# TMmichi/mujoco_jaco

Hardware: AMD Instinct MI355X
Metric: env-steps/sec at batch 65 536 (full Jaco + gripper + contacts) (higher is better)
Workload: dtype f32

## Files before the change

### __graft_entry__.py

```python
import os
import subprocess
import sys

ROOT = os.path.dirname(os.path.abspath(__file__))
CSRC = os.path.join(ROOT, "mujoco_jaco_amd", "csrc")
HIPCC = os.environ.get("HIPCC", "/opt/rocm/bin/hipcc")


D12 = ["-DJNB=13", "-DJNV=18", "-DJNQ=19", "-DJB0=12", "-DJB1=18", "-DJNSENS=64", "-DJMAXCHAIN=8", "-DJMAXDESC=12", "-DJMAXINNER=9"]
D30 = ["-DJNB=20", "-DJNV=30", "-DJNQ=32", "-DJB0=18", "-DJB1=24", "-DJNU=18", "-DJNSENS=40", "-DJMAXGEOM=128", "-DJMAXPAIR=3584", "-DJMAXINNER=12",
       "-DJMAXMPAIR=192", "-DJACO_LIGHT_WAVES=2"]


FLAGS = ["--offload-arch=gfx950", "-O3", "-std=c++17", "-fno-hip-fp32-correctly-rounded-divide-sqrt", "-fno-slp-vectorize",
         "-fgpu-flush-denormals-to-zero", "-fPIC", "-Rpass-analysis=kernel-resource-usage", "-I", os.path.join(CSRC, "include")]
NKERNEL_TU = 14


def _variant_jobs(name, extra):
    bdir = os.path.join(ROOT, "build", name)
    os.makedirs(bdir, exist_ok=True)
    jobs, objs = [], []
    for tu in list(range(NKERNEL_TU)) + [-1]:
        src = "jaco_env.hip" if tu < 0 else "kernels.hip"
# ... 34 lines not shown
    while todo or running:
        while todo and len(running) < workers and not failed:
            cmd, log = todo.pop(0)
            running.append((subprocess.Popen(cmd, cwd=CSRC, stdout=open(log, "w"), stderr=subprocess.STDOUT), cmd, log))
        if failed and not running:
            break
        p, cmd, log = running.pop(0)
        if p.poll() is None:
            running.append((p, cmd, log))
            import time
            time.sleep(0.2)
            continue
        if p.returncode == 0:
            open(log[:-4] + ".cmd", "w").write(" ".join(cmd))
        if p.returncode != 0:
            failed.append((cmd, log))
            for q, _, _ in running:
                q.terminate()
            for q, _, _ in running:
                q.wait()
            running = []
    if failed:
        cmd, log = failed[0]
        raise RuntimeError("hipcc failed: %s\n%s" % (" ".join(cmd), open(log).read()[-4000:]))
    for link in links:
        subprocess.check_call(link, cwd=CSRC)


VARIANTS = {
    "default": [],
    "d12": D12,
    "d30": D30,
    "prof": ["-DJACO_PROFILE_STAGES"],
}


def build():
    build_libs({k: v for k, v in VARIANTS.items() if k != "prof" or os.environ.get("JACO_BUILD_PROF") == "1"})
    subprocess.check_call(["make", "-s", "-C", os.path.join(ROOT, "oracle")])
    subprocess.check_call(["make", "-s", "-C", os.path.join(ROOT, "tests", "emu")])
    subprocess.check_call(["make", "-s", "-C", os.path.join(ROOT, "tests", "emu_osc")])
    subprocess.check_call(["make", "-s", "-C", os.path.join(ROOT, "tests", "emu_osc_task")])
    subprocess.check_call(["make", "-s", "-C", os.path.join(ROOT, "tests", "emu_joint")])
    if os.path.isdir("/root/reference/env_script/assets/jaco2") and not os.path.exists(
            os.path.join(ROOT, "mujoco_jaco_amd", "assets", "jaco2_curtain_torque.jacomdl")):
        subprocess.check_call([sys.executable, "-m", "mujoco_jaco_amd.modelc.compile"], cwd=ROOT)
    sys.path.insert(0, ROOT)
    import mujoco_jaco_amd
    from mujoco_jaco_amd import _lib
    _lib.load()
    _lib.load("_d12")
    _lib.load("_d30")


def smoke():
    sys.path.insert(0, ROOT)
    sys.path.insert(0, os.path.join(ROOT, "tests"))
    import numpy as np
    import torch
    from mujoco_jaco_amd import workload
    from mujoco_jaco_amd.modelc import blob
    from mujoco_jaco_amd.physics import BatchedMujoco
    from oracle_binding import Oracle

    B, nsub = 64, 20
    M = blob.load(os.path.join(ROOT, "mujoco_jaco_amd", "assets", "jaco2_curtain_torque.jacomdl"))
    q = workload.reset_states(M["qpos0"], B, seed=7, f32_draws=True)
    c = workload.random_ctrl(B, seed=8, scale=0.2).astype(np.float32).astype(np.float64)
    env = BatchedMujoco(B, device=0)
    dev = env.device
    env.set_state(torch.tensor(q, dtype=torch.float32, device=dev), None, None)
# ... 31 lines not shown
```

### mujoco_jaco_amd/csrc/physics_kernel.h

```cpp
#pragma once
#include <stdint.h>
#include <jaco/model_dev.h>
#include <jaco/wave_ops.h>

#ifndef JACO_WRENCH
#define JACO_WRENCH 0
#endif
template <int MAXEFC_, int MAXCON_, int MAXCAND_, bool CONTACT_ = true>
struct JacoCaps {
  static_assert(MAXEFC_ % 64 == 0, "rows are dealt out 64 at a time (one per lane): the row capacity must be a multiple of 64");
  static constexpr bool WRENCH = CONTACT_ && JACO_WRENCH != 0;
  static_assert(WRENCH || JMAXGEOM != 64 || JNV != 21 || MAXCAND_ <= MAXEFC_ * 25 - 520 - 256 - 576, "default layout: the candidate list must fit behind the geom poses in the constraint-row area");
  static constexpr int MAXEFC = MAXEFC_, MAXCON = MAXCON_, MAXCAND = MAXCAND_, NR = MAXEFC_ / 64;
  static constexpr bool CONTACT = CONTACT_;
  static constexpr int JROWS = CONTACT_ ? MAXEFC_ : (JNB <= 16 ? 16 : 32), NGEOM = CONTACT_ ? JMAXGEOM : 1;
  static_assert(CONTACT_ || JNB <= 32, "limit rows of the contact-free instantiation");
};
#if JACO_WRENCH
typedef JacoCaps<128, 32, 240> JacoLight;
#else
typedef JacoCaps<64, 32, 240> JacoLight;
#endif
typedef JacoCaps<128, 32, 512> JacoMedium;
#ifndef JACO_HEAVY_ROWS
// ... 14 lines not shown
#define JFLAG_CON_OVERFLOW 1u
#define JFLAG_EFC_OVERFLOW 2u
#define JFLAG_CAND_OVERFLOW 4u
#define JFLAG_NAN 8u
#define JFLAG_SOLVER_MAXITER 16u
#define JFLAG_HEAVY_TIER 32u
#define JFLAG_BAIL_CAUSE_SHIFT 8
#define JFLAG_TIER_RETURN 128u

#define JMINVAL 1e-15f
#define JTASK_FLOATS 40

#define JPROF_N 16
struct JProfCtx {
  unsigned long long tprev;
  unsigned long long* row;
};
#ifdef JACO_PROFILE_STAGES
JDEV void jprof_stamp(JProfCtx& pc, int i, int lane) {
  unsigned long long t = __builtin_amdgcn_s_memtime();
  if (lane == 0 && pc.row) pc.row[i] += t - pc.tprev;
  pc.tprev = __builtin_amdgcn_s_memtime();
}
#define JSTAMP(i) jprof_stamp(pc, (i), lane)
#else
#define JSTAMP(i)
#endif
#ifdef JACO_NARROW_PROFILE
#define JSTAMP_NEWTON(i) JSTAMP(6)
#define JSTAMP_NARROW(i) JSTAMP(i)
#else
#define JSTAMP_NEWTON(i) JSTAMP(i)
#define JSTAMP_NARROW(i)
#endif

struct JacoContactRec {
  float dist, pos[3], frame[9];
  float force[6];
  int geom[2], body[2], dim;
};
#define JCONREC_WORDS 24
#define JCONREC_MAX_CAPACITY 1024
#define JSTR_(x) #x
#define JSTR(x) JSTR_(x)
static inline const char* jaco_contact_record_check(const void* rec, const int* ncon, int capacity) {
  if (!ncon || capacity < 1 || capacity > JCONREC_MAX_CAPACITY) return "needs a count buffer and 1 <= capacity <= " JSTR(JCONREC_MAX_CAPACITY);
  if ((reinterpret_cast<uintptr_t>(rec) & 15u) != 0) return "the record buffer must be 16-byte aligned";
  return nullptr;
}

enum JacoMode { JM_CTRL = 0, JM_STEP = 1, JM_FORWARD = 2, JM_HOLD = 3, JM_TAKE_ACTION = 4, JM_TERMINAL = 5, JM_PREREACH = 6 };
#define JM_REAL_STEP(m) ((m) <= JM_STEP)
#define JM_MASKED(m) ((m) == JM_FORWARD || (m) == JM_HOLD || (m) == JM_PREREACH)
#define JM_TASK_SUBSTEPS(m) ((m) == JM_STEP || (m) == JM_HOLD || (m) == JM_PREREACH)
#define JM_NO_SUBSTEP(m) ((m) == JM_TAKE_ACTION || (m) == JM_TERMINAL)

struct JacoStepArgs {
  const JacoModelDev* model;
  const float* hull;
  float* qpos;
  float* qvel;
  float* qpos_lo;
  float* qvel_lo;
  float* qacc_ws;
  const float* ctrl;
  float* sensordata;
// ... 776 lines not shown
template <class L>
JDEV void stage_limit_rows(const JacoModelDev* m, L& s, int lane, const StagePrefetch& pf) {
  bool act = false;
  float dist = 0.f, sgn = 1.f;
  int d = 0;
  if (lane < m->nbody && s.mc.b_jtype[lane] == JJ_HINGE && pf.limited) {
    float q = s.qpos[s.mc.b_qadr[lane]];
    float lo = q - pf.lo, hi = pf.hi - q;
    d = s.mc.b_dadr[lane];
    if (lo < 0.f) { act = true; dist = lo; sgn = 1.f; }
    else if (hi < 0.f) { act = true; dist = hi; sgn = -1.f; }
  }
  unsigned long long mask = wave_ballot(act);
  int r = wave_prefix_count(mask);
  if (act) {
    if (L::Caps::WRENCH) {
      for (int k = 0; k < 8; k++) s.J[r * 8 + k] = 0.f;
      s.J[r * 8] = sgn;
    } else {
      for (int k = 0; k < JNV; k++) s.J[r * JLD + k] = 0.f;
      s.J[r * JLD + d] = sgn;
    }
    float R;
    s.e_aref[r] = row_params(m->b_solref[lane], m->b_solimp[lane], dist, sgn * s.qvel[d], m->d_invweight[d], &R);
    s.e_D[r] = 1.f / R;
    s.e_con[r] = ((d < JB0 ? 1 : (d < JB1 ? 2 : 4)) << 16) | (L::Caps::WRENCH ? (JW_UNIT | (d << 19)) : 0);
  }
  if (lane == 0) { s.nefc = popc64(mask); s.nlimit = s.nefc; }
}

struct NewtonOut { float qacc, qfrc_con, qdamped; int iters; bool have_qdamped; };
#define JDAMPED_BLOCKS 1

template <int NR>
JDEV void rows_dot(const float* J, const float (&jrow)[JNV], float vk, int lane, int ne, int nv, float (&out)[NR]) {
  float vb[JNV];
#pragma unroll
  for (int k = 0; k < JNV; k++) vb[k] = wave_bcast(vk, k);
  if (NR == 1) {
    float acc = 0.f;
#pragma unroll
    for (int k = 0; k < JNV; k++) acc += jrow[k] * vb[k];
    out[0] = acc;
    return;
  }
  const float* Jr[NR];
#pragma unroll
  for (int q = 0; q < NR; q++) { int r = lane + 64 * q; Jr[q] = J + (r < ne ? r : 0) * JLD; out[q] = 0.f; }
#pragma unroll
  for (int k = 0; k < JNV; k++) {
#pragma unroll
    for (int q = 0; q < NR; q++) out[q] += Jr[q][k] * vb[k];
  }
  (void)nv;
}
JDEV float mat_vec(const float (&mrow)[JNV], float vk) {
  float vb[JNV];
#pragma unroll
  for (int k = 0; k < JNV; k++) vb[k] = wave_bcast(vk, k);
  float acc = 0.f;
#pragma unroll
  for (int k = 0; k < JNV; k++) acc += mrow[k] * vb[k];
  return acc;
}
template <int NR>
JDEV float jt_vec(const float* J, const float (&f)[NR], int ne, int lane, int nv) {
  float acc = 0.f;
  int kk = lane < nv ? lane : 0;
#pragma unroll
  for (int q = 0; q < NR; q++) {
    int n = ne - 64 * q;
    n = n > 64 ? 64 : n;
    const float* Jq = J + (64 * q) * JLD + kk;
    int rl = 0;
    for (; rl + 4 <= n; rl += 4) {
      float j0 = Jq[(rl + 0) * JLD], j1 = Jq[(rl + 1) * JLD], j2 = Jq[(rl + 2) * JLD], j3 = Jq[(rl + 3) * JLD];
      const float f0 = wave_bcast(f[q], rl), f1 = wave_bcast(f[q], rl + 1), f2 = wave_bcast(f[q], rl + 2), f3 = wave_bcast(f[q], rl + 3);
      acc += j0 * f0 + j1 * f1 + j2 * f2 + j3 * f3;
    }
    for (; rl < n; rl++) acc += Jq[rl * JLD] * wave_bcast(f[q], rl);
  }
  return lane < nv ? acc : 0.f;
}

#ifndef JACO_NEWTON_LOOKAHEAD
#define JACO_NEWTON_LOOKAHEAD 1
#endif
JDEV bool newton_next_round_is_idle(bool any_row_switched, float al, float improvement, float scale, float tol) {
  const float r = 1.f - al;
  return JACO_NEWTON_LOOKAHEAD && !any_row_switched && r * r * improvement * scale < tol;
}
template <class L>
JDEV NewtonOut stage_newton(const JacoModelDev* m, L& s, const float (&mrow)[JNV], float smooth, float hd, int lane, JProfCtx& pc) {
  (void)pc;
  constexpr int NR = L::Caps::NR, MAXEFC = L::Caps::MAXEFC;
  NewtonOut out;
  int nv = m->nv, ne = wave_uniform_i(s.nefc);
  out.qfrc_con = 0.f; out.iters = 0; out.qdamped = 0.f; out.have_qdamped = false;
  float h0[JNV];
#pragma unroll
  for (int j = 0; j < JNV; j++) h0[j] = lane < nv ? mrow[j] : (lane == j ? 1.f : 0.f);
  const int blockmask = 1 | (nv > JB0 ? 2 : 0) | (nv > JB1 ? 4 : 0);
  if (ne == 0) {
    if (m->has_damping == 1) {
      out.qacc = ldl_block0_dual(h0, smooth, hd, lane, &out.qdamped) + ldl_solve_blocks(h0, smooth, lane, blockmask & 6);
      out.have_qdamped = true;
    } else out.qacc = ldl_solve_blocks(h0, smooth, lane, blockmask);
    return out;
  }
  if (ne > MAXEFC) ne = MAXEFC;
  bool valid[NR];
  float D[NR], ar[NR], x[NR], f[NR], jp[NR];
  int blk[NR];
  float jrow[JNV];
#pragma unroll
  for (int q = 0; q < NR; q++) {
    int r = lane + 64 * q;
    valid[q] = r < ne;
    D[q] = valid[q] ? s.e_D[r] : 0.f;
    ar[q] = valid[q] ? s.e_aref[r] : 0.f;
    blk[q] = valid[q] ? (s.e_con[r] >> 16) & 7 : 0;
  }
#pragma unroll
  for (int k = 0; k < JNV; k++) jrow[k] = (NR == 1 && lane < ne) ? s.J[lane * JLD + k] : 0.f;
  float scale = 1.f / (m->meaninertia * (float)(nv > 1 ? nv : 1));
  float tol = m->tolerance;
  int rowblk = 0;
#pragma unroll
  for (int q = 0; q < NR; q++) rowblk |= blk[q];
  const int rowblocks = (wave_ballot(rowblk & 1) ? 1 : 0) | (wave_ballot(rowblk & 2) ? 2 : 0) | (wave_ballot(rowblk & 4) ? 4 : 0);
  const bool mine = lane < nv && ((lane < JB0 ? 1 : (lane < JB1 ? 2 : 4)) & rowblocks) != 0;
  float afree;
  if ((rowblocks & 1) == 0 && m->has_damping == 1) {
    afree = ldl_block0_dual(h0, smooth, hd, lane, &out.qdamped);
    out.have_qdamped = true;
    afree += ldl_solve_blocks(h0, smooth, lane, ~rowblocks & 6 & blockmask);
  } else afree = ldl_solve_blocks(h0, smooth, lane, ~rowblocks & 7 & blockmask);
  float a = mine ? s.qacc_ws[lane] : afree;
  float Ma = mat_vec(mrow, a) - smooth;
  Ma = mine ? Ma : 0.f;
  rows_dot<NR>(s.J, jrow, a, lane, ne, nv, x);
#pragma unroll
  for (int q = 0; q < NR; q++) x[q] = valid[q] ? x[q] - ar[q] : 0.f;
  JSTAMP_NEWTON(11);
#ifdef JACO_EMULATED
  if (lane == 0) emu_counter[8]++;
#endif
  int it = 0, nls = 0;
  for (; it < m->iterations; it++) {
    lane = wave_opaque_i(lane);
#ifdef JACO_EMULATED
    if (lane == 0) emu_counter[9]++;
#endif
    bool coupled = false;
#pragma unroll
    for (int q = 0; q < NR; q++) {
      f[q] = x[q] < 0.f ? -D[q] * x[q] : 0.f;
      coupled = coupled || (x[q] < 0.f && (blk[q] & (blk[q] - 1)) != 0);
    }
    bool full = wave_ballot(coupled) != 0ull;
    float* xs = NR == 1 ? s.smooth : s.e_x;
#pragma unroll
    for (int q = 0; q < NR; q++) if (valid[q]) { s.e_f[lane + 64 * q] = x[q] < 0.f ? D[q] : 0.f; xs[lane + 64 * q] = x[q]; }
    wave_sync();
    float h[JNV], jtf;
    if ((rowblocks & 1) == 0) {
      acc16x16 C;
      acc_zero(C);
      const int uq = lane >> 4, col = lane & 15;
      const float cj = col < JNV - JB0 ? 1.f : 0.f, cx = col == JNV - JB0 ? -1.f : 0.f;
      const float* jcol = s.J + JB0 + (col < JNV - JB0 ? col : 0);
      const int last = ne - 1;
      for (int r0 = 0; r0 < ne; r0 += 16) {
        float jv[4], wv[4];
#pragma unroll
        for (int u = 0; u < 4; u++) {
          const int r = r0 + 4 * u + uq, rc = r < last ? r : last;
          jv[u] = cj * jcol[rc * JLD] + cx * xs[rc];
          wv[u] = r < ne ? s.e_f[rc] : 0.f;
// ... 14 lines not shown
    } else {
    acc32x32 C;
    acc_zero(C);
    const int uh = lane >> 5, col = lane & 31;
    const float cj = col < JNV ? 1.f : 0.f, cx = col == JNV ? -1.f : 0.f;
    const float* jcol = s.J + (col < JNV ? col : 0);
    const int last = ne - 1;
    for (int r0 = 0; r0 < ne; r0 += 8) {
      float jv[4], wv[4];
#pragma unroll
      for (int u = 0; u < 4; u++) {
        const int r = r0 + 2 * u + uh, rc = r < last ? r : last;
        jv[u] = cj * jcol[rc * JLD] + cx * xs[rc];
        wv[u] = r < ne ? s.e_f[rc] : 0.f;
      }
#pragma unroll
      for (int u = 0; u < 4; u++) wave_mfma_32x32x2(jv[u], wv[u] * jv[u], C);
    }
    JSTAMP_NEWTON(12);
#pragma unroll
    for (int j2 = 0; j2 < JNV; j2++) {
      const int reg = (j2 & 3) + 4 * (j2 >> 3);
      float cv = ((j2 >> 2) & 1) ? wave_shfl(C.v[reg], (lane + 32) & 63) : C.v[reg];
      h[j2] = lane < nv ? mrow[j2] + cv : (lane == j2 ? 1.f : 0.f);
    }
    jtf = ((JNV >> 2) & 1) ? wave_shfl(C.v[(JNV & 3) + 4 * (JNV >> 3)], (lane + 32) & 63) : C.v[(JNV & 3) + 4 * (JNV >> 3)];
    }
    float grad = Ma - (lane < nv ? jtf : 0.f);
    float gn = sqrtf(wave_sum(grad * grad));
    if (gn * scale < tol) break;
    float p = !full ? ldl_solve_blocks(h, -grad, lane, rowblocks) : ((rowblocks & 1) == 0 ? ldl_block<JB0, JNV>(h, -grad, lane) : ldl_solve<true>(h, -grad, lane));
    p = lane < nv ? p : 0.f;
    JSTAMP_NEWTON(13);
    float Mp = mat_vec(mrow, p);
    float pMp, pMa;
    wave_sum2(p * Mp, p * Ma, &pMp, &pMa);
    rows_dot<NR>(s.J, jrow, p, lane, ne, nv, jp);
#pragma unroll
    for (int q = 0; q < NR; q++) jp[q] = valid[q] ? jp[q] : 0.f;
    float al = 0.f, lo = 0.f, hi = 3.0e38f, d10 = 0.f, dlo = 0.f, dhi = 0.f;
    for (int ls = 0; ls < m->ls_iterations; ls++) {
      float s1 = 0.f, s2 = 0.f;
#pragma unroll
      for (int q = 0; q < NR; q++) {
        float xa = x[q] + al * jp[q];
        s1 += xa < 0.f ? D[q] * xa * jp[q] : 0.f;
        s2 += xa < 0.f ? D[q] * jp[q] * jp[q] : 0.f;
      }
      float w1, w2;
      wave_sum2(s1, s2, &w1, &w2);
      float d1 = pMa + al * pMp + w1, d2 = pMp + w2;
      if (ls == 0) d10 = fabsf(d1);
#ifdef JACO_TRACE_LS
      if (lane == 0) printf("it %d ls %d al %.9g d1 %.6g d2 %.6g lo %.9g hi %.9g pMa %.6g pMp %.6g\n", it, ls, al, d1, d2, lo, hi, pMa, pMp);
#endif
      if (ls > 0 && fabsf(d1) <= 1e-6f * d10) break;
      if (d1 < 0.f) { lo = al; dlo = -d1; } else { hi = al; dhi = d1; }
      if (hi < 1.0e38f && fmaxf(dlo, dhi) * (hi - lo) * scale < 1e-3f * tol) break;
      const float stepn = d1 / d2;
      float nx = al - stepn;
      if (!(nx > lo && nx < hi)) nx = hi < 1.0e38f ? 0.5f * (lo + hi) : 2.f * al + 1.f;
      if (nx == al) break;
      al = nx;
      nls++;
    }
    float dc = 0.f;
    bool switched = false;
#pragma unroll
    for (int q = 0; q < NR; q++) {
      float dx = al * jp[q], xn = x[q] + dx;
      bool was = x[q] < 0.f, is = xn < 0.f;
      switched = switched || was != is;
      dc += (was && is) ? 0.5f * D[q] * dx * (2.f * x[q] + dx) : (is ? 0.5f * D[q] * xn * xn : (was ? -0.5f * D[q] * x[q] * x[q] : 0.f));
      x[q] = xn;
    }
    const bool any_switched = wave_ballot(switched) != 0ull;
    float improvement = -(al * pMa + 0.5f * al * al * pMp + wave_sum(dc));
    JSTAMP_NEWTON(14);
    a += al * p; Ma += al * Mp;
    if (improvement * scale < tol || newton_next_round_is_idle(any_switched, al, improvement, scale, tol)) { it++; break; }
  }
#pragma unroll
  for (int q = 0; q < NR; q++) f[q] = x[q] < 0.f ? -D[q] * x[q] : 0.f;
  out.qacc = a;
  out.qfrc_con = jt_vec<NR>(s.J, f, ne, lane, nv);
  out.iters = it | (nls << 8);
#pragma unroll
  for (int q = 0; q < NR; q++) if (valid[q]) s.e_f[lane + 64 * q] = f[q];
  return out;
}

struct WCol { sv S; unsigned mv; };
template <class L>
JDEV WCol wcol_load(const L& s, int col, int nv) {
  WCol c;
  const bool ok = col < nv;
  c.S = ldsv(s.cdof[ok ? col : 0]);
  if (!ok) { c.S.a = mk3(0.f, 0.f, 0.f); c.S.b = mk3(0.f, 0.f, 0.f); }
  c.mv = ok ? s.mc.b_descmask[s.mc.d_body[col]] << 1 : 0u;
  return c;
}
JDEV float wrow_entry(const WCol& c, int col, const v4& a, const v4& b, int con) {
  const float sgn = (float)((int)((c.mv >> ((con >> 24) & 31)) & 1u) - (int)((c.mv >> ((con >> 19) & 31)) & 1u));
  const float body = sgn * (a.x * c.S.a.x + a.y * c.S.a.y + a.z * c.S.a.z + a.w * c.S.b.x + b.x * c.S.b.y + b.y * c.S.b.z);
  return (con & JW_UNIT) ? (((con >> 19) & 31) == col ? a.x : 0.f) : body;
}
template <int NR, class L>
JDEV void rows_dot_w(L& s, const float (&w)[NR][6], const int (&con)[NR], float vk, int lane, int nv, int ncon, float (&out)[NR]) {
  float* vs = s.smooth + 32;
  wave_sync();
  if (lane < nv) vs[lane] = vk;
  wave_sync();
  for (int idx = lane; idx < 6 * ncon; idx += 64) {
    const int c = idx / 6, comp = idx - 6 * c, obs = s.c_ob[c];
    const int B1 = (obs >> 8) & 31, B2 = (obs >> 24) & 31;
    const unsigned m1 = B1 ? s.mc.b_chain[B1 - 1] : 0u, m2 = B2 ? s.mc.b_chain[B2 - 1] : 0u;
    const unsigned plus = m2 & ~m1;
    unsigned mask = m1 ^ m2;
    float acc = 0.f;
    while (mask) {
      const int k = __builtin_ctz(mask);
      mask &= mask - 1u;
      const float t = s.cdof[k][comp] * vs[k];
      acc += ((plus >> k) & 1u) ? t : -t;
    }
    s.c_frame[c][3 + comp] = acc;
  }
  wave_sync();
#pragma unroll
  for (int q = 0; q < NR; q++) {
    const bool unit = (con[q] & JW_UNIT) != 0;
    const float* Dc = s.c_frame[unit ? 0 : (con[q] & 255)] + 3;
    float acc = 0.f;
#pragma unroll
    for (int c = 0; c < 6; c++) acc += w[q][c] * Dc[c];
    out[q] = unit ? w[q][0] * vs[(con[q] >> 19) & 31] : acc;
  }
}

template <class L>
JDEV NewtonOut stage_newton_w(const JacoModelDev* m, L& s, const float (&mrow)[JNV], float smooth, float hd, int lane, JProfCtx& pc) {
  (void)pc;
  constexpr int NR = L::Caps::NR, MAXEFC = L::Caps::MAXEFC;
  NewtonOut out;
  const int nv = m->nv, ncon = wave_uniform_i(s.ncon), nlim = wave_uniform_i(s.nlimit);
  int ne = wave_uniform_i(s.nefc);
  out.qfrc_con = 0.f; out.iters = 0; out.qdamped = 0.f; out.have_qdamped = false;
  float h0[JNV];
#pragma unroll
  for (int j = 0; j < JNV; j++) h0[j] = lane < nv ? mrow[j] : (lane == j ? 1.f : 0.f);
  const int blockmask = 1 | (nv > JB0 ? 2 : 0) | (nv > JB1 ? 4 : 0);
  if (ne == 0) {
    if (m->has_damping == 1) {
      out.qacc = ldl_block0_dual(h0, smooth, hd, lane, &out.qdamped) + ldl_solve_blocks(h0, smooth, lane, blockmask & 6);
      out.have_qdamped = true;
    } else out.qacc = ldl_solve_blocks(h0, smooth, lane, blockmask);
    return out;
  }
  if (ne > MAXEFC) ne = MAXEFC;
  bool valid[NR];
  float D[NR], ar[NR], x[NR], f[NR], jp[NR], w[NR][6];
  int con[NR];
#pragma unroll
  for (int q = 0; q < NR; q++) {
    const int r = lane + 64 * q;
    valid[q] = r < ne;
    const int rc = valid[q] ? r : 0;
    D[q] = valid[q] ? s.e_D[rc] : 0.f;
    ar[q] = valid[q] ? s.e_aref[rc] : 0.f;
    con[q] = valid[q] ? s.e_con[rc] : 0;
    const v4 a = ld4(s.J + 8 * rc), b = ld4(s.J + 8 * rc + 4);
    w[q][0] = valid[q] ? a.x : 0.f; w[q][1] = valid[q] ? a.y : 0.f; w[q][2] = valid[q] ? a.z : 0.f;
    w[q][3] = valid[q] ? a.w : 0.f; w[q][4] = valid[q] ? b.x : 0.f; w[q][5] = valid[q] ? b.y : 0.f;
  }
// ... 129 lines not shown
#pragma unroll
    for (int q = 0; q < NR; q++) {
      float dx = al * jp[q], xn = x[q] + dx;
      bool was = x[q] < 0.f, is = xn < 0.f;
      switched = switched || was != is;
      dc += (was && is) ? 0.5f * D[q] * dx * (2.f * x[q] + dx) : (is ? 0.5f * D[q] * xn * xn : (was ? -0.5f * D[q] * x[q] * x[q] : 0.f));
      x[q] = xn;
    }
    const bool any_switched = wave_ballot(switched) != 0ull;
    float improvement = -(al * pMa + 0.5f * al * al * pMp + wave_sum(dc));
    JSTAMP_NEWTON(14);
    a += al * p; Ma += al * Mp;
    if (improvement * scale < tol || newton_next_round_is_idle(any_switched, al, improvement, scale, tol)) { it++; break; }
  }
#pragma unroll
  for (int q = 0; q < NR; q++) f[q] = x[q] < 0.f ? -D[q] * x[q] : 0.f;
  out.qacc = a;
  out.iters = it | (nls << 8);
  wave_sync();
#pragma unroll
  for (int q = 0; q < NR; q++) if (valid[q]) { s.e_f[lane + 64 * q] = f[q]; s.J[8 * (lane + 64 * q) + JW_WT] = f[q]; }
  wave_sync();
  for (int ci = lane; ci < ncon; ci += 64) {
    const int cd = s.c_dim[ci], nrow = cd == 1 ? 1 : 2 * (cd - 1), r0 = s.c_efc[ci];
    float F[6] = {0.f, 0.f, 0.f, 0.f, 0.f, 0.f};
    for (int e = 0; e < nrow; e++) {
      const v4 ra = ld4(s.J + 8 * (r0 + e)), rb = ld4(s.J + 8 * (r0 + e) + 4);
      F[0] += rb.z * ra.x; F[1] += rb.z * ra.y; F[2] += rb.z * ra.z; F[3] += rb.z * ra.w; F[4] += rb.z * rb.x; F[5] += rb.z * rb.y;
    }
#pragma unroll
    for (int c = 0; c < 6; c++) s.c_frame[ci][3 + c] = F[c];
  }
  wave_sync();
  {
    const WCol own = wcol_load(s, lane, nv);
    float acc = 0.f;
    for (int c = 0; c < ncon; c++) {
      const int obs = s.c_ob[c];
      const float sgn = (float)((int)((own.mv >> ((obs >> 24) & 31)) & 1u) - (int)((own.mv >> ((obs >> 8) & 31)) & 1u));
      const float* F = s.c_frame[c] + 3;
      acc += sgn * (F[0] * own.S.a.x + F[1] * own.S.a.y + F[2] * own.S.a.z + F[3] * own.S.b.x + F[4] * own.S.b.y + F[5] * own.S.b.z);
    }
    for (int r = 0; r < nlim; r++) {
      const int cn = s.e_con[r];
      if (((cn >> 19) & 31) == lane) acc += s.J[8 * r] * s.J[8 * r + JW_WT];
    }
    out.qfrc_con = lane < nv ? acc : 0.f;
  }
  return out;
}

template <class L>
JDEV NewtonOut stage_newton_limits(const JacoModelDev* m, L& s, const float (&mrow)[JNV], float smooth, float hd, int lane) {
  NewtonOut out;
  const int nv = m->nv, ne = wave_uniform_i(s.nefc);
  out.qfrc_con = 0.f; out.iters = 0; out.qdamped = 0.f; out.have_qdamped = false;
  float h0[JNV];
#pragma unroll
  for (int j = 0; j < JNV; j++) h0[j] = lane < nv ? mrow[j] : (lane == j ? 1.f : 0.f);
  const int blockmask = 1 | (nv > JB0 ? 2 : 0) | (nv > JB1 ? 4 : 0);
  if (ne == 0) {
    if (m->has_damping == 1) {
      out.qacc = ldl_block0_dual(h0, smooth, hd, lane, &out.qdamped) + ldl_solve_blocks(h0, smooth, lane, blockmask & 6);
      out.have_qdamped = true;
    } else out.qacc = ldl_solve_blocks(h0, smooth, lane, blockmask);
    return out;
  }
// ... 94 lines not shown
      const float e1 = q1 * cm1 + q0 * d1 + q2 * d3 - q3 * d2;
      const float e2 = q2 * cm1 + q0 * d2 - q1 * d3 + q3 * d1;
      const float e3 = q3 * cm1 + q0 * d3 + q1 * d2 - q2 * d1;
      if (comp) {
        f2 r;
        r = comp_add(q0, l0, e0, 0.f); q0 = r.hi; l0 = r.lo;
        r = comp_add(q1, l1, e1, 0.f); q1 = r.hi; l1 = r.lo;
        r = comp_add(q2, l2, e2, 0.f); q2 = r.hi; l2 = r.lo;
        r = comp_add(q3, l3, e3, 0.f); q3 = r.hi; l3 = r.lo;
      } else { q0 += e0; q1 += e1; q2 += e2; q3 += e3; }
    }
    const float r2 = fmaf(q3, q3, fmaf(q2, q2, fmaf(q1, q1, fmaf(q0, q0, -1.f)))) + 2.f * (q0 * l0 + q1 * l1 + q2 * l2 + q3 * l3);
    if (comp && fabsf(r2) < 1e-3f) {
      const float k = r2 * (-0.5f + 0.375f * r2);
      f2 r;
      r = comp_add(q0, l0, q0 * k, 0.f); q0 = r.hi; l0 = r.lo;
      r = comp_add(q1, l1, q1 * k, 0.f); q1 = r.hi; l1 = r.lo;
      r = comp_add(q2, l2, q2 * k, 0.f); q2 = r.hi; l2 = r.lo;
      r = comp_add(q3, l3, q3 * k, 0.f); q3 = r.hi; l3 = r.lo;
    } else {
      const float n = sqrtf(q0 * q0 + q1 * q1 + q2 * q2 + q3 * q3);
      if (n < JMINVAL) { q0 = 1.f; q1 = q2 = q3 = 0.f; } else { const float in = 1.f / n; q0 *= in; q1 *= in; q2 *= in; q3 *= in; }
      l0 = l1 = l2 = l3 = 0.f;
    }
    s.qpos[qa + 3] = q0; s.qpos[qa + 4] = q1; s.qpos[qa + 5] = q2; s.qpos[qa + 6] = q3;
    if (comp) { s.qpos_lo[qa + 3] = l0; s.qpos_lo[qa + 4] = l1; s.qpos_lo[qa + 5] = l2; s.qpos_lo[qa + 6] = l3; }
  }
}

#include "collision.h"
#include "env_logic.h"

template <class L>
JDEV void newton_side(const JacoModelDev* m, L& s, const float (&mrow)[JNV], float smooth, int lane, NewtonOut& out) {
  float* sd = side_buf(s);
  int ns = wave_uniform_i(s.nside);
  ns = ns < 0 ? 0 : (ns > JSIDE_ROWS ? JSIDE_ROWS : ns);
  const int nv = m->nv;
  const bool mine = lane >= JB1 && lane < JNV, vr = lane < ns;
  const int kk = mine ? lane - JB1 : 0, rr = vr ? lane : 0;
  float js[6];
#pragma unroll
  for (int k = 0; k < 6; k++) js[k] = vr ? sd[JSIDE_J + rr * 6 + k] : 0.f;
  const float D = vr ? sd[JSIDE_D + rr] : 0.f, ar = vr ? sd[JSIDE_AREF + rr] : 0.f;
  const float scale = 1.f / (m->meaninertia * (float)(nv > 1 ? nv : 1)), tol = m->tolerance;
  wave_sync();
  float a = mine ? s.qacc_ws[lane] : 0.f;
  float Ma = 0.f, x = 0.f;
#pragma unroll
  for (int j = 0; j < 6; j++) { const float aj = wave_bcast(a, JB1 + j); Ma += mrow[JB1 + j] * aj; x += js[j] * aj; }
  Ma = mine ? Ma - smooth : 0.f;
  x = vr ? x - ar : 0.f;
  float jtf = 0.f;
  int it = 0;
  for (; it < m->iterations; it++) {
    lane = wave_opaque_i(lane);
    if (vr) { sd[JSIDE_F + lane] = x < 0.f ? D : 0.f; sd[JSIDE_AREF + lane] = x < 0.f ? -D * x : 0.f; }
    wave_sync();
    float h[JNV];
#pragma unroll
    for (int j = 0; j < JNV; j++) h[j] = (j >= JB1 && mine) ? mrow[j] : 0.f;
    jtf = 0.f;
    for (int r = 0; r < ns; r++) {
      const float* Jr = sd + JSIDE_J + r * 6;
      const float jk = Jr[kk], t = sd[JSIDE_F + r] * jk;
      jtf += jk * sd[JSIDE_AREF + r];
#pragma unroll
// ... 10 lines not shown
    Mp = mine ? Mp : 0.f;
    jp = vr ? jp : 0.f;
    float pMp, pMa;
    wave_sum2(p * Mp, p * Ma, &pMp, &pMa);
    float al = 0.f, lo = 0.f, hi = 3.0e38f, d10 = 0.f, dlo = 0.f, dhi = 0.f;
    for (int ls = 0; ls < m->ls_iterations; ls++) {
      const float xa = x + al * jp;
      const float s1 = xa < 0.f ? D * xa * jp : 0.f, s2 = xa < 0.f ? D * jp * jp : 0.f;
      float w1, w2;
      wave_sum2(s1, s2, &w1, &w2);
      float d1 = pMa + al * pMp + w1, d2 = pMp + w2;
      if (ls == 0) d10 = fabsf(d1);
      if (ls > 0 && fabsf(d1) <= 1e-6f * d10) break;
      if (d1 < 0.f) { lo = al; dlo = -d1; } else { hi = al; dhi = d1; }
      if (hi < 1.0e38f && fmaxf(dlo, dhi) * (hi - lo) * scale < 1e-3f * tol) break;
      float nx = al - d1 / d2;
      if (!(nx > lo && nx < hi)) nx = hi < 1.0e38f ? 0.5f * (lo + hi) : 2.f * al + 1.f;
      if (nx == al) break;
      al = nx;
    }
    const float dx = al * jp, xn = x + dx;
    const bool was = x < 0.f, is = xn < 0.f;
    const bool any_switched = wave_ballot(was != is) != 0ull;
    const float dc = (was && is) ? 0.5f * D * dx * (2.f * x + dx) : (is ? 0.5f * D * xn * xn : (was ? -0.5f * D * x * x : 0.f));
    x = xn;
    const float improvement = -(al * pMa + 0.5f * al * al * pMp + wave_sum(dc));
    a += al * p; Ma += al * Mp;
    if (improvement * scale < tol || newton_next_round_is_idle(any_switched, al, improvement, scale, tol)) { it++; break; }
  }
  const float f = x < 0.f ? -D * x : 0.f;
  wave_sync();
  if (vr) sd[JSIDE_F + lane] = f;
  wave_sync();
  float qf = 0.f;
  for (int r = 0; r < ns; r++) qf += sd[JSIDE_J + r * 6 + kk] * sd[JSIDE_F + r];
  out.qacc = mine ? a : out.qacc;
  out.qfrc_con = mine ? qf : out.qfrc_con;
  if (it > (out.iters & 255)) out.iters = (out.iters & ~255) | (it & 255);
}

JDEV void queue_push(const JacoStepArgs& A, int t, int env, int left, int lane) {
  if (lane == 0) st_wt_i(&A.remaining[env], left);
  dev_stores_done();
  wave_sync();
  if (lane == 0) {
    int slot = jaco_atomic_inc(A.q[t].count);
    st_wt_i(&A.q[t].list[slot], env);
    dev_stores_done();
  }
}
JDEV void hint_raise(const JacoStepArgs& A, int env, int tier, int lane) {
  if (lane == 0 && A.hint) atomicMax(&A.hint[env], tier);
}

template <class L>
JDEV void stage_record(const JacoModelDev* m, L& s, JacoContactRec* rec, int* nout, int cap, int env, int lane) {
  const int ncon = L::Caps::CONTACT ? wave_uniform_i(s.ncon) : 0;
  if (lane == 0) nout[env] = ncon;
  if constexpr (L::Caps::CONTACT) {
    const int n = ncon < cap ? ncon : cap;
    for (int ci = lane; ci < n; ci += 64) {
      const int cd = s.c_dim[ci], nrow = cd == 1 ? 1 : 2 * (cd - 1), r0 = s.c_efc[ci], obs = s.c_ob[ci];
      const float* f = (SideRows<L>::on && r0 >= JSIDE_BASE) ? side_buf(s) + JSIDE_F + (r0 - JSIDE_BASE) : s.e_f + r0;
      const JacoPairParam& P = m->pair[s.c_pair[ci]];
      float fc[6] = {0.f, 0.f, 0.f, 0.f, 0.f, 0.f};
      for (int e = 0; e < nrow; e++) fc[0] += f[e];
#pragma unroll
      for (int k = 1; k < 6; k++) if (k < cd) fc[k] = P.mu[k - 1] * (f[2 * k - 2] - f[2 * k - 1]);
      const float* fr = s.c_frame[ci];
      v4* o = reinterpret_cast<v4*>(rec + (size_t)env * cap + ci);
// ... 236 lines not shown
    if (!LIGHT) {
      constexpr int LCON = TIER == 3 ? JacoHeavy::MAXCON : (TIER == 2 ? JacoMedium::MAXCON : JacoLight::MAXCON);
      constexpr int LEFC = TIER == 3 ? JacoHeavy::MAXEFC : (TIER == 2 ? JacoMedium::MAXEFC : JacoLight::MAXEFC);
      constexpr int LCAND = TIER == 3 ? JacoHeavy::MAXCAND : (TIER == 2 ? JacoMedium::MAXCAND : JacoLight::MAXCAND);
      const bool rows_fit = s.nefc <= LEFC || (TIER == 1 && SideRows<JacoLDS<JacoLight>>::on && s.nside_cand > 0 && s.nefc - s.nside_cand <= LEFC);
      const bool fits = s.ncon <= LCON && rows_fit && s.nsphere <= LCAND;
      calm = fits ? calm + 1 : 0;
      if (!fits && !tier_used) { tier_used = true; if (A.hint_mode != 2) hint_raise(A, env, TIER, lane); }
    }
    if (TIER == 3) flags |= cflags;
    if (TIER < 3 && cflags) {
      left = nsub - sub;
      bailed = true;
      flags |= (cflags & 7u) << (JFLAG_BAIL_CAUSE_SHIFT + 3 * TIER);
      if (JM_TASK_SUBSTEPS(emode)) {
        if (lane < nu) s.task[JT_CTRL + lane] = s.ctrl[lane];
        if (lane == 0) { s.task[JT_PENDING] = 1.f; s.task[JT_SUB] = (float)sub; }
        wave_sync();
      }
      break;
    }
    float mrow[JNV], h[JNV];
    {
      const int blo = lane < JB0 ? 0 : (lane < JB1 ? JB0 : JB1), bn = lane < JB0 ? JB0 : (lane < JB1 ? JB1 - JB0 : JNV - JB1);
      const int rbase = lane < nv ? m_index(lane, blo) : 0;
#pragma unroll
      for (int j = 0; j < JNV; j++) { const bool in = lane < nv && j >= blo && j < blo + bn; mrow[j] = in ? s.M[in ? rbase + j - blo : 0] : 0.f; }
    }
    float smooth = lane < nv ? s.smooth[lane] : 0.f;
    float qas = 0.f;
    wave_sync();
    const float hdamp = (m->has_damping && lane < nv) ? m->timestep * pf.damping : 0.f;
    NewtonOut nw;
    if constexpr (C::WRENCH) nw = stage_newton_w(m, s, mrow, smooth, hdamp, lane, pc);
    else if constexpr (C::CONTACT) nw = stage_newton(m, s, mrow, smooth, hdamp, lane, pc);
    else nw = stage_newton_limits(m, s, mrow, smooth, hdamp, lane);
    if (SideRows<JacoLDS<C>>::on) { if (wave_uniform_i(s.nside) > 0) newton_side(m, s, mrow, smooth, lane, nw); }
    JSTAMP(6);
    iters = nw.iters & 255;
    int nls_dbg = nw.iters >> 8;
    nls_last = nls_dbg;
    if (iters >= m->iterations) flags |= JFLAG_SOLVER_MAXITER;
    wave_sync();
    if (C::CONTACT) stage_touch(m, s, lane, &sens);
    JSTAMP(7);
    float total = smooth + nw.qfrc_con, qacc_e = nw.qacc;
    if (m->has_damping) {
      float qd;
      if (nw.have_qdamped) qd = nw.qdamped;
      else {
#pragma unroll
        for (int j = 0; j < JNV; j++) h[j] = (lane < nv ? mrow[j] : 0.f) + (lane == j ? (lane < nv ? hdamp : 1.f) : 0.f);
        qd = ldl_solve_blocks(h, total, lane, JDAMPED_BLOCKS);
      }
      qacc_e = lane < JB0 ? qd : nw.qacc;
    }
    if (A.dbg && env == A.dbg_env && sub == nsub - 1) {
      float* D = A.dbg;
      if (lane < m->nbody) {
        for (int k = 0; k < 3; k++) D[JDBG_XPOS + 3 * lane + k] = s.xpos[lane][k];
        for (int k = 0; k < 9; k++) D[JDBG_XMAT + 9 * lane + k] = s.xmat[lane][k];
      }
      for (int i = lane; i < JNV * JNV; i += 64) {
        const int d = i / JNV, j = i % JNV;
        const bool same = (d < JB0) == (j < JB0) && (d < JB1) == (j < JB1);
        D[JDBG_M + i] = same ? s.M[m_index(d, j)] : 0.f;
      }
      if (lane < nv) {
        D[JDBG_BIAS + lane] = s.bias[lane]; D[JDBG_SMOOTH + lane] = smooth; D[JDBG_QACC_SMOOTH + lane] = qas;
        D[JDBG_QACC + lane] = nw.qacc; D[JDBG_QFRC_CON + lane] = nw.qfrc_con;
      }
      if (lane == 0) { D[JDBG_NCON] = (float)s.ncon; D[JDBG_NCON + 1] = (float)(s.nefc + s.nside); D[JDBG_NCON + 2] = (float)iters; D[JDBG_NCON + 3] = (float)s.ncand; }
      for (int c = lane; c < s.ncon && c < JDBG_MAXCON; c += 64) {
        float* o = D + JDBG_CONTACT + 8 * c;
        o[0] = s.c_dist[c]; o[1] = s.c_pos[c][0]; o[2] = s.c_pos[c][1]; o[3] = s.c_pos[c][2];
        o[4] = s.c_frame[c][0]; o[5] = s.c_frame[c][1]; o[6] = s.c_frame[c][2]; o[7] = (float)s.c_pair[c];
      }
      for (int r = lane; r < s.nefc && r < JDBG_MAXEFC; r += 64) {
        float* o = D + JDBG_EFC + 4 * r;
        o[0] = s.e_aref[r]; o[1] = 1.f / s.e_D[r]; o[2] = 0.f; o[3] = s.e_f[r];
      }
      if (lane < s.ncon) D[JDBG_CFN + lane] = s.c_fn[lane];
      if (lane < m->nsensor) D[JDBG_SENS + lane] = sens;
    }
    wave_sync();
    if (emode == JM_FORWARD || fwd) break;
    if (lane < nv) {
      float v;
      if (m->compensated) {
        const f2 nvl = comp_advance(s.qvel[lane], s.qvel_lo[lane], m->timestep, m->timestep_lo, qacc_e, 0.f);
// ... 468 lines not shown
```

Before: 2.034 million.

## Skip arm-block work in Newton when no constraint rows touch block 0

When no active constraint rows touch the arm block (block 0), the Newton solver now skips the block-0 broadcasts and dot products in mat_vec and rows_dot, and does not load the block-0 columns of J. It also skips computing qfrc_con (J^T f) when the damped path already provides qdamped and no debug dump is requested. This removes redundant wave broadcasts and multiply-adds in the inner iteration loop and the final reduction. The risk is correctness if the free-only regime assumption is wrong, and extra branches or register pressure. Census and no-regime build variants are added for analysis.

```diff
diff --git a/__graft_entry__.py b/__graft_entry__.py
--- a/__graft_entry__.py
+++ b/__graft_entry__.py
@@ -90,11 +90,14 @@
     "d12": D12,
     "d30": D30,
     "prof": ["-DJACO_PROFILE_STAGES"],
+    "noregime": ["-DJACO_NEWTON_REGIME=0"],
+    "census": ["-DJACO_PROFILE_STAGES", "-DJACO_REGIME_CENSUS"],
 }
+PRODUCT = ("default", "d12", "d30")
 
 
 def build():
-    build_libs({k: v for k, v in VARIANTS.items() if k != "prof" or os.environ.get("JACO_BUILD_PROF") == "1"})
+    build_libs({k: v for k, v in VARIANTS.items() if k in PRODUCT or (k == "prof" and os.environ.get("JACO_BUILD_PROF") == "1")})
     subprocess.check_call(["make", "-s", "-C", os.path.join(ROOT, "oracle")])
     subprocess.check_call(["make", "-s", "-C", os.path.join(ROOT, "tests", "emu")])
     subprocess.check_call(["make", "-s", "-C", os.path.join(ROOT, "tests", "emu_osc")])
diff --git a/mujoco_jaco_amd/csrc/physics_kernel.h b/mujoco_jaco_amd/csrc/physics_kernel.h
--- a/mujoco_jaco_amd/csrc/physics_kernel.h
+++ b/mujoco_jaco_amd/csrc/physics_kernel.h
@@ -70,6 +70,13 @@
 #else
 #define JSTAMP_NEWTON(i) JSTAMP(i)
 #define JSTAMP_NARROW(i)
+#endif
+#ifdef JACO_REGIME_CENSUS
+#undef JSTAMP
+#define JSTAMP(i)
+#define JCENSUS(ne, rowblocks, dual) do { if (lane == 0 && pc.row) { pc.row[0] += 1; if (((rowblocks) & 1) == 0) { pc.row[1] += 1; pc.row[2] += (dual) ? 1 : 0; pc.row[3] += (ne); } } } while (0)
+#else
+#define JCENSUS(ne, rowblocks, dual)
 #endif
 
 struct JacoContactRec {
@@ -912,35 +919,48 @@
 struct NewtonOut { float qacc, qfrc_con, qdamped; int iters; bool have_qdamped; };
 #define JDAMPED_BLOCKS 1
 
+#ifndef JACO_NEWTON_REGIME
+#define JACO_NEWTON_REGIME 1
+#endif
 template <int NR>
-JDEV void rows_dot(const float* J, const float (&jrow)[JNV], float vk, int lane, int ne, int nv, float (&out)[NR]) {
-  float vb[JNV];
-#pragma unroll
-  for (int k = 0; k < JNV; k++) vb[k] = wave_bcast(vk, k);
-  if (NR == 1) {
-    float acc = 0.f;
-#pragma unroll
-    for (int k = 0; k < JNV; k++) acc += jrow[k] * vb[k];
-    out[0] = acc;
-    return;
-  }
+JDEV void rows_dot(const float* J, const float (&jrow)[JNV], float vk, int lane, int ne, int nv, float (&out)[NR], bool free_only = false) {
   const float* Jr[NR];
 #pragma unroll
   for (int q = 0; q < NR; q++) { int r = lane + 64 * q; Jr[q] = J + (r < ne ? r : 0) * JLD; out[q] = 0.f; }
-#pragma unroll
-  for (int k = 0; k < JNV; k++) {
-#pragma unroll
-    for (int q = 0; q < NR; q++) out[q] += Jr[q][k] * vb[k];
+  if (!(JACO_NEWTON_REGIME && free_only)) {
+    float vb[JB0];
+#pragma unroll
+    for (int k = 0; k < JB0; k++) vb[k] = wave_bcast(vk, k);
+#pragma unroll
+    for (int k = 0; k < JB0; k++) {
+#pragma unroll
+      for (int q = 0; q < NR; q++) out[q] += (NR == 1 ? jrow[k] : Jr[q][k]) * vb[k];
+    }
+  }
+  float vb[JNV - JB0];
+#pragma unroll
+  for (int k = JB0; k < JNV; k++) vb[k - JB0] = wave_bcast(vk, k);
+#pragma unroll
+  for (int k = JB0; k < JNV; k++) {
+#pragma unroll
+    for (int q = 0; q < NR; q++) out[q] += (NR == 1 ? jrow[k] : Jr[q][k]) * vb[k - JB0];
   }
   (void)nv;
 }
-JDEV float mat_vec(const float (&mrow)[JNV], float vk) {
-  float vb[JNV];
-#pragma unroll
-  for (int k = 0; k < JNV; k++) vb[k] = wave_bcast(vk, k);
+JDEV float mat_vec(const float (&mrow)[JNV], float vk, bool free_only = false) {
   float acc = 0.f;
-#pragma unroll
-  for (int k = 0; k < JNV; k++) acc += mrow[k] * vb[k];
+  if (!(JACO_NEWTON_REGIME && free_only)) {
+    float vb[JB0];
+#pragma unroll
+    for (int k = 0; k < JB0; k++) vb[k] = wave_bcast(vk, k);
+#pragma unroll
+    for (int k = 0; k < JB0; k++) acc += mrow[k] * vb[k];
+  }
+  float vb[JNV - JB0];
+#pragma unroll
+  for (int k = JB0; k < JNV; k++) vb[k - JB0] = wave_bcast(vk, k);
+#pragma unroll
+  for (int k = JB0; k < JNV; k++) acc += mrow[k] * vb[k - JB0];
   return acc;
 }
 template <int NR>
@@ -970,8 +990,11 @@
   const float r = 1.f - al;
   return JACO_NEWTON_LOOKAHEAD && !any_row_switched && r * r * improvement * scale < tol;
 }
+JDEV bool newton_qfrc_wanted(const JacoModelDev* m, const NewtonOut& out, bool dump) {
+  return !JACO_NEWTON_REGIME || dump || (m->has_damping && !out.have_qdamped);
+}
 template <class L>
-JDEV NewtonOut stage_newton(const JacoModelDev* m, L& s, const float (&mrow)[JNV], float smooth, float hd, int lane, JProfCtx& pc) {
+JDEV NewtonOut stage_newton(const JacoModelDev* m, L& s, const float (&mrow)[JNV], float smooth, float hd, int lane, JProfCtx& pc, bool dump) {
   (void)pc;
   constexpr int NR = L::Caps::NR, MAXEFC = L::Caps::MAXEFC;
   NewtonOut out;
@@ -1001,8 +1024,6 @@
     ar[q] = valid[q] ? s.e_aref[r] : 0.f;
     blk[q] = valid[q] ? (s.e_con[r] >> 16) & 7 : 0;
   }
-#pragma unroll
-  for (int k = 0; k < JNV; k++) jrow[k] = (NR == 1 && lane < ne) ? s.J[lane * JLD + k] : 0.f;
   float scale = 1.f / (m->meaninertia * (float)(nv > 1 ? nv : 1));
   float tol = m->tolerance;
   int rowblk = 0;
@@ -1010,6 +1031,16 @@
   for (int q = 0; q < NR; q++) rowblk |= blk[q];
   const int rowblocks = (wave_ballot(rowblk & 1) ? 1 : 0) | (wave_ballot(rowblk & 2) ? 2 : 0) | (wave_ballot(rowblk & 4) ? 4 : 0);
   const bool mine = lane < nv && ((lane < JB0 ? 1 : (lane < JB1 ? 2 : 4)) & rowblocks) != 0;
+  const bool free_only = JACO_NEWTON_REGIME && (rowblocks & 1) == 0;
+#pragma unroll
+  for (int k = 0; k < JNV; k++) jrow[k] = 0.f;
+  if (NR == 1 && !free_only) {
+#pragma unroll
+    for (int k = 0; k < JB0; k++) jrow[k] = lane < ne ? s.J[lane * JLD + k] : 0.f;
+  }
+#pragma unroll
+  for (int k = JB0; k < JNV; k++) jrow[k] = (NR == 1 && lane < ne) ? s.J[lane * JLD + k] : 0.f;
+  JCENSUS(ne, rowblocks, m->has_damping == 1);
   float afree;
   if ((rowblocks & 1) == 0 && m->has_damping == 1) {
     afree = ldl_block0_dual(h0, smooth, hd, lane, &out.qdamped);
@@ -1017,14 +1048,14 @@
     afree += ldl_solve_blocks(h0, smooth, lane, ~rowblocks & 6 & blockmask);
   } else afree = ldl_solve_blocks(h0, smooth, lane, ~rowblocks & 7 & blockmask);
   float a = mine ? s.qacc_ws[lane] : afree;
-  float Ma = mat_vec(mrow, a) - smooth;
+  float Ma = mat_vec(mrow, a, free_only) - smooth;
   Ma = mine ? Ma : 0.f;
-  rows_dot<NR>(s.J, jrow, a, lane, ne, nv, x);
+  rows_dot<NR>(s.J, jrow, a, lane, ne, nv, x, free_only);
 #pragma unroll
   for (int q = 0; q < NR; q++) x[q] = valid[q] ? x[q] - ar[q] : 0.f;
   JSTAMP_NEWTON(11);
 #ifdef JACO_EMULATED
-  if (lane == 0) emu_counter[8]++;
+  if (lane == 0) { emu_counter[8]++; if ((rowblocks & 1) == 0) emu_counter[11]++; }
 #endif
   int it = 0, nls = 0;
   for (; it < m->iterations; it++) {
@@ -1105,10 +1136,10 @@
     float p = !full ? ldl_solve_blocks(h, -grad, lane, rowblocks) : ((rowblocks & 1) == 0 ? ldl_block<JB0, JNV>(h, -grad, lane) : ldl_solve<true>(h, -grad, lane));
     p = lane < nv ? p : 0.f;
     JSTAMP_NEWTON(13);
-    float Mp = mat_vec(mrow, p);
+    float Mp = mat_vec(mrow, p, free_only);
     float pMp, pMa;
     wave_sum2(p * Mp, p * Ma, &pMp, &pMa);
-    rows_dot<NR>(s.J, jrow, p, lane, ne, nv, jp);
+    rows_dot<NR>(s.J, jrow, p, lane, ne, nv, jp, free_only);
 #pragma unroll
     for (int q = 0; q < NR; q++) jp[q] = valid[q] ? jp[q] : 0.f;
     float al = 0.f, lo = 0.f, hi = 3.0e38f, d10 = 0.f, dlo = 0.f, dhi = 0.f;
@@ -1156,7 +1187,10 @@
 #pragma unroll
   for (int q = 0; q < NR; q++) f[q] = x[q] < 0.f ? -D[q] * x[q] : 0.f;
   out.qacc = a;
-  out.qfrc_con = jt_vec<NR>(s.J, f, ne, lane, nv);
+  if (newton_qfrc_wanted(m, out, dump)) out.qfrc_con = jt_vec<NR>(s.J, f, ne, lane, nv);
+#ifdef JACO_EMULATED
+  if (lane == 0 && newton_qfrc_wanted(m, out, dump)) emu_counter[12]++;
+#endif
   out.iters = it | (nls << 8);
 #pragma unroll
   for (int q = 0; q < NR; q++) if (valid[q]) s.e_f[lane + 64 * q] = f[q];
@@ -1212,7 +1246,7 @@
 }
 
 template <class L>
-JDEV NewtonOut stage_newton_w(const JacoModelDev* m, L& s, const float (&mrow)[JNV], float smooth, float hd, int lane, JProfCtx& pc) {
+JDEV NewtonOut stage_newton_w(const JacoModelDev* m, L& s, const float (&mrow)[JNV], float smooth, float hd, int lane, JProfCtx& pc, bool dump) {
   (void)pc;
   constexpr int NR = L::Caps::NR, MAXEFC = L::Caps::MAXEFC;
   NewtonOut out;
@@ -1408,7 +1442,7 @@
     for (int c = 0; c < 6; c++) s.c_frame[ci][3 + c] = F[c];
   }
   wave_sync();
-  {
+  if (newton_qfrc_wanted(m, out, dump)) {
     const WCol own = wcol_load(s, lane, nv);
     float acc = 0.f;
     for (int c = 0; c < ncon; c++) {
@@ -1569,7 +1603,7 @@
 #include "env_logic.h"
 
 template <class L>
-JDEV void newton_side(const JacoModelDev* m, L& s, const float (&mrow)[JNV], float smooth, int lane, NewtonOut& out) {
+JDEV void newton_side(const JacoModelDev* m, L& s, const float (&mrow)[JNV], float smooth, int lane, NewtonOut& out, bool dump) {
   float* sd = side_buf(s);
   int ns = wave_uniform_i(s.nside);
   ns = ns < 0 ? 0 : (ns > JSIDE_ROWS ? JSIDE_ROWS : ns);
@@ -1646,10 +1680,12 @@
   wave_sync();
   if (vr) sd[JSIDE_F + lane] = f;
   wave_sync();
-  float qf = 0.f;
-  for (int r = 0; r < ns; r++) qf += sd[JSIDE_J + r * 6 + kk] * sd[JSIDE_F + r];
   out.qacc = mine ? a : out.qacc;
-  out.qfrc_con = mine ? qf : out.qfrc_con;
+  if (newton_qfrc_wanted(m, out, dump)) {
+    float qf = 0.f;
+    for (int r = 0; r < ns; r++) qf += sd[JSIDE_J + r * 6 + kk] * sd[JSIDE_F + r];
+    out.qfrc_con = mine ? qf : out.qfrc_con;
+  }
   if (it > (out.iters & 255)) out.iters = (out.iters & ~255) | (it & 255);
 }
 
@@ -1952,10 +1988,11 @@
     wave_sync();
     const float hdamp = (m->has_damping && lane < nv) ? m->timestep * pf.damping : 0.f;
     NewtonOut nw;
-    if constexpr (C::WRENCH) nw = stage_newton_w(m, s, mrow, smooth, hdamp, lane, pc);
-    else if constexpr (C::CONTACT) nw = stage_newton(m, s, mrow, smooth, hdamp, lane, pc);
+    const bool dump = A.dbg && env == A.dbg_env && sub == nsub - 1;
+    if constexpr (C::WRENCH) nw = stage_newton_w(m, s, mrow, smooth, hdamp, lane, pc, dump);
+    else if constexpr (C::CONTACT) nw = stage_newton(m, s, mrow, smooth, hdamp, lane, pc, dump);
     else nw = stage_newton_limits(m, s, mrow, smooth, hdamp, lane);
-    if (SideRows<JacoLDS<C>>::on) { if (wave_uniform_i(s.nside) > 0) newton_side(m, s, mrow, smooth, lane, nw); }
+    if (SideRows<JacoLDS<C>>::on) { if (wave_uniform_i(s.nside) > 0) newton_side(m, s, mrow, smooth, lane, nw, dump); }
     JSTAMP(6);
     iters = nw.iters & 255;
     int nls_dbg = nw.iters >> 8;
@@ -1972,10 +2009,13 @@
 #pragma unroll
         for (int j = 0; j < JNV; j++) h[j] = (lane < nv ? mrow[j] : 0.f) + (lane == j ? (lane < nv ? hdamp : 1.f) : 0.f);
         qd = ldl_solve_blocks(h, total, lane, JDAMPED_BLOCKS);
+#ifdef JACO_EMULATED
+        if (lane == 0) emu_counter[13]++;
+#endif
       }
       qacc_e = lane < JB0 ? qd : nw.qacc;
     }
-    if (A.dbg && env == A.dbg_env && sub == nsub - 1) {
+    if (dump) {
       float* D = A.dbg;
       if (lane < m->nbody) {
         for (int k = 0; k < 3; k++) D[JDBG_XPOS + 3 * lane + k] = s.xpos[lane][k];
```

Result: faster. 2.069 million, median of 6 (+1.7%).
